# modelscope/FunCodec

Hardware: NVIDIA H100
Metric: codec frames/sec (encode+RVQ+decode) (higher is better)
Workload: dtype f32

## Files before the change

funcodec_b200/csrc/conv_tc.cu:

```cuda
#include <cuda.h>
#include "common.cuh"
#include "kernels.h"
#include "tc_sm90.cuh"
#include <stdlib.h>

namespace fcb {

using namespace tc;

constexpr int TC_M = 128;
constexpr int TC_KC = 32;
constexpr int TC_THREADS = 640;
constexpr int TC_RAW_MAX = 8;
constexpr int TC_PROD = 128;
constexpr int TC_PROWS = TC_PROD / 8;
constexpr int TC_A_ROWS_MAX = 144;
constexpr int TC_GROUP_MMAS = 48;
constexpr int TC_LAUNCH_REGS = 96, TC_PROD_REGS = 96, TC_CTL_REGS = 64, TC_CONS_REGS = 112;
static_assert(128 * (2 * TC_CONS_REGS + 2 * TC_PROD_REGS + TC_CTL_REGS) <= TC_THREADS * TC_LAUNCH_REGS, "register pool");

__device__ __forceinline__ float elu_fast(float v) { return v > 0.f ? v : (__expf(v) - 1.0f); }
__device__ __forceinline__ float elu_scaled(float vs, float k, float s) { return vs > 0.f ? vs : fmaf(exp2f_approx(vs * k), s, -s); }

struct TcSmemLayout {
    int a_rows;
    int a_stage;
    int b_stage;
    int na, nb;
    int nraw, raw_slot, raw_in1, raw_cf;
    int off_b, off_raw, off_bar, total;
};

__host__ __device__ inline TcSmemLayout tc_layout(int K, int S, int n_tile, int na, int nb, int nraw = 0, int raw_pitch = 128,
                                                   int has1 = 0) {
    TcSmemLayout L;
    const int qmax = (K - 1) / S;
    L.a_rows = ((TC_M + qmax + 7) / 8) * 8;
    L.a_stage = 2 * L.a_rows * 128;
    L.b_stage = 2 * n_tile * 128;
    L.na = na; L.nb = nb;
    L.off_b = na * L.a_stage;
    L.nraw = nraw;
    L.raw_in1 = L.a_rows * raw_pitch;
    L.raw_cf = (1 + has1) * L.a_rows * raw_pitch;
    L.raw_slot = (L.raw_cf + 512 + 127) / 128 * 128;
    L.off_raw = L.off_b + nb * L.b_stage;
    L.off_bar = L.off_raw + nraw * L.raw_slot;
    L.total = L.off_bar + 8 * (2 * na + 2 * nb + 2 * TC_RAW_MAX) + 160;
    return L;
}

__host__ __device__ inline int tc_units_per_group(int K, int S, int group_mmas) {
    const int taps = (K + S - 1) / S;
    int g = group_mmas / (12 * taps);
    return g < 1 ? 1 : g;
}

struct TcArgs {
    TcSmemLayout L;
    int na, nb, n_tiles, w_resident, nraw;
    int n_chunks, n_sc, split, n_units, upg, n_groups, n_tt, n_nt, units_per_tile, tq_rows, raw_pitch;
};

struct TcTile { int b, nt, tt; };

__device__ __forceinline__ TcTile tc_tile(int id, int n_nt, int n_tt) {
    TcTile t;
    t.nt = id % n_nt;
    const int r = id / n_nt;
    t.tt = r % n_tt;
    t.b = r / n_tt;
    return t;
}

template <int N_TILE, int KSTEPS>
__device__ __forceinline__ void tc_issue_tap(float (&acc)[N_TILE / 2], uint32_t a_hi, uint32_t a_lo, uint32_t b_hi, uint32_t b_lo,
                                             uint32_t accum) {
    wgmma_fence();
#pragma unroll
    for (int ks = 0; ks < KSTEPS; ++ks) {
        WgmmaF16<N_TILE>::mma(acc, make_desc_k_sw128(a_lo + ks * 32), make_desc_k_sw128(b_hi + ks * 32), ks == 0 ? accum : 1u);
        WgmmaF16<N_TILE>::mma(acc, make_desc_k_sw128(a_hi + ks * 32), make_desc_k_sw128(b_lo + ks * 32), 1u);
        WgmmaF16<N_TILE>::mma(acc, make_desc_k_sw128(a_hi + ks * 32), make_desc_k_sw128(b_hi + ks * 32), 1u);
    }
    wgmma_commit();
}

template <int N_TILE, bool FREQ>
__global__ void __launch_bounds__(TC_THREADS, 1) conv1d_tc_kernel(const __grid_constant__ ConvParams p, const __grid_constant__ TcArgs ka,
                                                                 const __grid_constant__ CUtensorMap tm0,
                                                                 const __grid_constant__ CUtensorMap tm1) {
    extern __shared__ __align__(1024) uint8_t smem_raw[];
    const int tid = threadIdx.x, lane = tid & 31, warp = tid >> 5;
    const int C_in = p.C_in, K = p.K, S = p.S;
    const bool has1 = p.in1.x != nullptr;
    const TcSmemLayout& L = ka.L;
#define na_stages ka.na
#define nb_stages ka.nb
#define n_tiles ka.n_tiles
#define w_resident ka.w_resident
#define nraw ka.nraw
#define raw_pitch ka.raw_pitch
#define n_chunks ka.n_chunks
#define n_sc ka.n_sc
#define n_units ka.n_units
#define upg ka.upg
#define n_groups ka.n_groups
#define n_tt ka.n_tt
#define n_nt ka.n_nt
    const bool split = ka.split != 0;

    uint8_t* smA = smem_raw;
    uint8_t* smB = smem_raw + L.off_b;
    uint64_t* bars = reinterpret_cast<uint64_t*>(smem_raw + L.off_bar);
    uint64_t* a_full = bars;
    uint64_t* a_empty = a_full + na_stages;
    uint64_t* b_full = a_empty + na_stages;
    uint64_t* b_empty = b_full + nb_stages;
    uint64_t* raw_full = b_empty + nb_stages;
    uint64_t* raw_empty = raw_full + TC_RAW_MAX;
    double* red = reinterpret_cast<double*>(raw_empty + TC_RAW_MAX);
    uint8_t* smR = smem_raw + L.off_raw;
#define units_per_tile ka.units_per_tile
#define tq_rows ka.tq_rows
    auto tile_interior = [&](int t0) -> bool {
        if (nraw == 0) return false;
        const int t_last = (t0 + TC_M < p.T_out ? t0 + TC_M : p.T_out) - 1;
        const int lo = t0 * S - p.pad_l;
        const int hi = t_last * S - p.pad_l + (K - 1);
        return lo >= 0 && hi < tq_rows * S;
    };

    if (tid == 0) {
        for (int i = 0; i < na_stages; ++i) { mbar_init(a_full + i, split ? 2 * TC_PROD : TC_PROD); mbar_init(a_empty + i, 2); }
        for (int i = 0; i < nb_stages; ++i) { mbar_init(b_full + i, 1); mbar_init(b_empty + i, 2); }
        for (int i = 0; i < TC_RAW_MAX; ++i) { mbar_init(raw_full + i, 1); mbar_init(raw_empty + i, TC_PROD); }
        mbar_fence_init();
    }
    __syncthreads();

    const int role = warp >> 2;
    if (role < 2) {
        setmaxnreg_dec<TC_PROD_REGS>();
        const int grp = role;
        const int ptid = tid & (TC_PROD - 1);
        const int jchunk = ptid & 7;
        const int wq = (ptid >> 5), lq = (lane >> 3);
        const int rsub = ((wq >> 1) << 3) + ((wq & 1) << 1) + (lq & 1) + ((lq >> 1) << 2);
        constexpr int NR = TC_A_ROWS_MAX / TC_PROWS;
        const int gt_max = (p.T_out - 1) * S - p.pad_l + (K - 1);
        const int step = split ? 1 : 2;
        const int half = split ? grp : 0;
        int tile = blockIdx.x, unit = split ? 0 : grp;
        int as = unit % na_stages;
        uint32_t aphase = 0;
        const float in_scale = p.tc_in_scale;
        int rawbase = 0;
        while (unit >= n_units && tile < n_tiles) {
            if (tile_interior(tc_tile(tile, n_nt, n_tt).tt * TC_M)) rawbase += units_per_tile;
            unit -= n_units; tile += gridDim.x;
        }
        while (tile < n_tiles) {
            const TcTile tl = tc_tile(tile, n_nt, n_tt);
            const int t0 = tl.tt * TC_M;
            int b = tl.b, f_out = 0;
            if (FREQ) { b = tl.b / p.fq.F_out; f_out = tl.b - b * p.fq.F_out; }
            const int pitch = FREQ ? p.fq.cin : C_in;
            const float* x0 = p.in0.x + (long long)b * p.in0.clip_stride + (long long)p.in0.row_off * pitch;
            const float* x1 = has1 ? p.in1.x + (long long)b * p.in1.clip_stride + (long long)p.in1.row_off * pitch : nullptr;
            const float* cf0 = p.in0.coef ? p.in0.coef + (long long)b * 2 * pitch : nullptr;
            const float* cf1 = (has1 && p.in1.coef) ? p.in1.coef + (long long)b * 2 * pitch : nullptr;
            const int cur_tile = tile;
            const bool interior = tile_interior(t0);
            for (; unit < n_units && tile == cur_tile; ) {
                const int sc = unit / S, ph = unit - sc * S;
                const int chunk = 2 * sc + half;
                const uint32_t par = aphase ^ 1;
                uint8_t* hi = smA + as * L.a_stage;
                uint8_t* lo = hi + L.a_rows * 128;
                const uint32_t c16 = (uint32_t)(half * 4 + (jchunk >> 1)), sub8 = (uint32_t)((jchunk & 1) << 3);
                if (p.dbg & 512) {
                    if (p.dbg & 64) mbar_wait(a_empty + as, par); else mbar_wait_backoff(a_empty + as, par, 64);
                } else if (chunk >= n_chunks) {
                    if (p.dbg & 64) mbar_wait(a_empty + as, par); else mbar_wait_backoff(a_empty + as, par, 64);
                } else if (interior) {
// ... 109 lines not shown
#pragma unroll
                    for (int j = 0; j < PB; ++j) {
                        const int u = rsub + TC_PROWS * (i0 + j);
                        if (u < L.a_rows) {
                            float4 v = make_float4(0.f, 0.f, 0.f, 0.f);
                            if (p.dbg & 2) v = xa[j];
                            else if (okr[j]) {
                                const float4 xv = xa[j];
                                v.x = fmaf(xv.x, a0.x, b0.x); v.y = fmaf(xv.y, a0.y, b0.y);
                                v.z = fmaf(xv.z, a0.z, b0.z); v.w = fmaf(xv.w, a0.w, b0.w);
                                if (has1) {
                                    const float4 yv = xb[j];
                                    v.x = v.x + fmaf(yv.x, a1.x, b1.x); v.y = v.y + fmaf(yv.y, a1.y, b1.y);
                                    v.z = v.z + fmaf(yv.z, a1.z, b1.z); v.w = v.w + fmaf(yv.w, a1.w, b1.w);
                                }
                                if (p.elu) {
                                    v.x = elu_scaled(v.x, p.tc_elu_k, in_scale); v.y = elu_scaled(v.y, p.tc_elu_k, in_scale);
                                    v.z = elu_scaled(v.z, p.tc_elu_k, in_scale); v.w = elu_scaled(v.w, p.tc_elu_k, in_scale);
                                }
                            }
                            if (p.dbg & 4) continue;
                            uint2 h, l;
                            split_f16x2(v.x, v.y, h.x, l.x);
                            split_f16x2(v.z, v.w, h.y, l.y);
                            const uint32_t o = (uint32_t)u * 128u + ((c16 ^ (uint32_t)(u & 7)) << 4) + sub8;
                            *reinterpret_cast<uint2*>(hi + o) = h;
                            *reinterpret_cast<uint2*>(lo + o) = l;
                        }
                    }
                }
                fence_proxy_async_smem();
                }
                mbar_arrive(a_full + as);
                as += step;
                if (as >= na_stages) { as -= na_stages; aphase ^= 1; }
                unit += step;
            }
            while (unit >= n_units && tile < n_tiles) {
                if (tile_interior(tc_tile(tile, n_nt, n_tt).tt * TC_M)) rawbase += units_per_tile;
                unit -= n_units; tile += gridDim.x;
            }
        }
    } else if (role == 2) {
        setmaxnreg_dec<TC_CTL_REGS>();
        if (warp == 8 && lane == 0) {
            const uint32_t bytes = (uint32_t)L.b_stage;
            int bs = 0;
            uint32_t bphase = 0;
            bool first = true;
            for (int tile = blockIdx.x; tile < n_tiles; tile += gridDim.x) {
                if (w_resident && !first) break;
                const TcTile tl = tc_tile(tile, n_nt, n_tt);
                const uint8_t* wbase = reinterpret_cast<const uint8_t*>(p.w_tc) + (long long)tl.nt * n_sc * K * bytes;
                int chunk = 0, ph = 0;
                for (int unit = 0; unit < n_units; ++unit) {
                    for (int k = ph; k < K; k += S) {
                        if (!w_resident) { if (p.dbg & 64) mbar_wait(b_empty + bs, bphase ^ 1); else mbar_wait_backoff(b_empty + bs, bphase ^ 1, 64); }
                        if (p.dbg & 256) { mbar_arrive(b_full + bs); }
                        else {
                            mbar_arrive_expect_tx(b_full + bs, bytes);
                            bulk_g2s(smB + bs * L.b_stage, wbase + ((long long)chunk * K + k) * bytes, bytes, b_full + bs);
                        }
                        if (++bs == nb_stages) { bs = 0; bphase ^= 1; }
                    }
                    if (++ph == S) { ph = 0; ++chunk; }
                }
                first = false;
            }
        } else if (warp == 9 && lane == 0 && nraw > 0 && !(p.dbg & 512)) {
            const uint32_t row_bytes = (uint32_t)(L.a_rows * raw_pitch);
            const uint32_t cbytes = (uint32_t)raw_pitch;
            const uint32_t n_cf = (p.in0.coef ? 2u : 0u) + ((has1 && p.in1.coef) ? 2u : 0u);
            const uint32_t unit_bytes = row_bytes * (has1 ? 2u : 1u) + n_cf * cbytes;
            int rc = 0;
            for (int tile = blockIdx.x; tile < n_tiles; tile += gridDim.x) {
                const TcTile tl = tc_tile(tile, n_nt, n_tt);
                const int t0 = tl.tt * TC_M;
                if (!tile_interior(t0)) continue;
                int b = tl.b, f_out = 0;
                if (FREQ) { b = tl.b / p.fq.F_out; f_out = tl.b - b * p.fq.F_out; }
                const int pitch = FREQ ? p.fq.cin : C_in;
                const float* cf0 = p.in0.coef ? p.in0.coef + (long long)b * 2 * pitch : nullptr;
                const float* cf1 = (has1 && p.in1.coef) ? p.in1.coef + (long long)b * 2 * pitch : nullptr;
                for (int sc = 0; sc < n_sc; ++sc)
                    for (int ph = 0; ph < S; ++ph) {
                        const int r = ph - p.pad_l;
                        const int fd = (r >= 0) ? r / S : -((-r + S - 1) / S);
                        const int tq0 = t0 + fd, php = r - fd * S;
                        for (int hh = 0; hh < 2; ++hh) {
                            const int chunk = 2 * sc + hh;
                            if (chunk >= n_chunks) break;
                            const int slot = rc % nraw;
                            mbar_wait(raw_empty + slot, (uint32_t)((rc / nraw) & 1) ^ 1);
                            uint8_t* dst = smR + slot * L.raw_slot;
                            mbar_arrive_expect_tx(raw_full + slot, unit_bytes);
                            int c0 = chunk * TC_KC;
                            if (FREQ) {
                                const int kf = c0 / pitch;
                                c0 -= kf * pitch;
                                int f_src = f_out * p.fq.SF + kf - p.fq.pad_f;
                                if (!p.pad_zero) f_src = reflect_index(f_src, p.fq.F_in);
                                tma_load_5d(dst, &tm0, c0, php, tq0, f_src, b, raw_full + slot);
                                if (has1) tma_load_5d(dst + L.raw_in1, &tm1, c0, php, tq0, f_src, b, raw_full + slot);
                            } else {
                                tma_load_4d(dst, &tm0, c0, php, tq0, b, raw_full + slot);
                                if (has1) tma_load_4d(dst + L.raw_in1, &tm1, c0, php, tq0, b, raw_full + slot);
                            }
                            if (cf0) {
                                bulk_g2s(dst + L.raw_cf, cf0 + c0, cbytes, raw_full + slot);
                                bulk_g2s(dst + L.raw_cf + 128, cf0 + pitch + c0, cbytes, raw_full + slot);
                            }
                            if (cf1) {
                                bulk_g2s(dst + L.raw_cf + 256, cf1 + c0, cbytes, raw_full + slot);
                                bulk_g2s(dst + L.raw_cf + 384, cf1 + pitch + c0, cbytes, raw_full + slot);
                            }
                            ++rc;
                        }
                    }
            }
        }
    } else {
        setmaxnreg_inc<TC_CONS_REGS>();
        constexpr int NA = N_TILE / 2;
        const int cw = warp - 12;
        const int wg = cw >> 2;
        const int ctid = tid - 12 * 32;
        const bool leader = (tid & 127) == 0;
        const uint32_t a_base = smem_u32(smA) + (uint32_t)(wg * 64 * 128), b_base = smem_u32(smB);
        const int r_lo = wg * 64 + (cw & 3) * 16 + (lane >> 2);
        const int cq = 2 * (lane & 3);
        const bool plain_out = FREQ && p.fq.FR == 1 && p.fq.TR == 1 && p.fq.c_store == p.C_out;
        const float out_scale = p.tc_out_scale;
        int fin_clip = -1, fin_local = 0;
        auto fin_flush = [&]() {
            if (fin_clip < 0 || fin_local == 0) return;
            int* flag = reinterpret_cast<int*>(red + 16);
            if (ctid == 0) {
                __threadfence();
                const int old = atomicAdd(p.fin_counter + fin_clip, fin_local);
                *flag = (old + fin_local == p.fin_parts) ? 1 : 0;
            }
            asm volatile("bar.sync 1, 256;" ::: "memory");
            const bool last_cta = *flag != 0;
            if (last_cta) {
                __threadfence();
                const double* pp = p.partials + (long long)fin_clip * p.fin_parts * 2;
                double fs = 0.0, fss = 0.0;
                for (int i = ctid; i < p.fin_parts; i += 256) { fs += __ldcg(pp + 2 * i); fss += __ldcg(pp + 2 * i + 1); }
#pragma unroll
                for (int o = 16; o > 0; o >>= 1) {
                    fs += __shfl_xor_sync(0xffffffffu, fs, o);
                    fss += __shfl_xor_sync(0xffffffffu, fss, o);
                }
                asm volatile("bar.sync 1, 256;" ::: "memory");
                if (lane == 0) { red[cw * 2] = fs; red[cw * 2 + 1] = fss; }
                asm volatile("bar.sync 1, 256;" ::: "memory");
                double ts = 0.0, tss = 0.0;
#pragma unroll
                for (int w = 0; w < 8; ++w) { ts += red[2 * w]; tss += red[2 * w + 1]; }
                const double mean_d = ts / p.fin_count;
                double var = tss / p.fin_count - mean_d * mean_d;
                if (var < 0.0) var = 0.0;
                const float mean = (float)mean_d, rstd = (float)(1.0 / sqrt(var + (double)p.fin_eps));
                if (ctid == 0) {
                    p.fin_stats[2 * fin_clip] = mean;
                    p.fin_stats[2 * fin_clip + 1] = rstd;
                    p.fin_counter[fin_clip] = 0;
                }
                if (p.fin_coef)
// ... 29 lines not shown
                        const uint32_t b_hi0 = b_base + bs * L.b_stage;
                        const uint32_t b_lo0 = b_hi0 + N_TILE * 128;
                        if (full_stage) tc_issue_tap<N_TILE, 4>(acc, a_hi0 + q * 128, a_lo0 + q * 128, b_hi0, b_lo0, accum);
                        else tc_issue_tap<N_TILE, 2>(acc, a_hi0 + q * 128, a_lo0 + q * 128, b_hi0, b_lo0, accum);
                        accum = 1;
                        wgmma_wait<1>();
                        mbar_arrive_if(b_empty + pend_b, leader && pend_b >= 0);
                        mbar_arrive_if(a_empty + pend_a, leader && pend_a >= 0);
                        pend_b = w_resident ? -1 : bs;
                        pend_a = -1;
                        if (++bs == nb_stages) { bs = 0; bphase ^= 1; }
                    }
                    pend_a = as;
                    if (++as == na_stages) { as = 0; aphase ^= 1; }
                    if (++ph == S) ph = 0;
                }
                wgmma_wait<0>();
                reg_fence(acc);
                if (leader) {
                    if (pend_b >= 0) mbar_arrive(b_empty + pend_b);
                    if (pend_a >= 0) mbar_arrive(a_empty + pend_a);
                }
                pend_a = -1; pend_b = -1;
#pragma unroll
                for (int i = 0; i < NA; ++i) tot[i] = g == 0 ? acc[i] : tot[i] + acc[i];
            }
            first = false;
            long long frow = 0;
            if (FREQ) {
                const int fb = tl.b / p.fq.F_out, ff = tl.b - fb * p.fq.F_out;
                frow = ((long long)fb * p.fq.F_out * p.fq.FR + (long long)ff * p.fq.FR) * ((long long)p.T_out * p.fq.TR);
            }
            const float* bias = p.bias + tl.nt * N_TILE;
            float s = 0.f, ss = 0.f;
#pragma unroll
            for (int j = 0; j < N_TILE / 8; ++j) {
                const int c = 8 * j + cq;
                const float bias0 = __ldg(bias + c), bias1 = __ldg(bias + c + 1);
#pragma unroll
                for (int h = 0; h < 2; ++h) {
                    const int t = tl.tt * TC_M + r_lo + 8 * h;
                    if (t >= p.T_out) continue;
                    float2 o;
                    o.x = fmaf(tot[4 * j + 2 * h], out_scale, bias0);
                    o.y = fmaf(tot[4 * j + 2 * h + 1], out_scale, bias1);
                    s += o.x + o.y;
                    ss = fmaf(o.x, o.x, ss); ss = fmaf(o.y, o.y, ss);
                    if (p.dbg & 8) continue;
                    if (!FREQ || plain_out) {
                        *reinterpret_cast<float2*>(p.out + (long long)tl.b * p.out_clip_stride + (long long)t * p.C_out + tl.nt * N_TILE + c) = o;
                    } else {
#pragma unroll
                        for (int e = 0; e < 2; ++e) {
                            const int co = tl.nt * N_TILE + c + e;
                            const int phs = co / p.fq.Cc, cch = co - phs * p.fq.Cc;
                            if (cch < p.fq.c_store) {
                                const int pf = phs / p.fq.TR, pt = phs - pf * p.fq.TR;
                                p.out[(frow + (long long)t * p.fq.TR + (long long)pf * p.T_out * p.fq.TR + pt) * p.fq.c_store + cch] = e ? o.y : o.x;
                            }
                        }
                    }
                }
            }
            if (p.partials && !(p.dbg & 16)) {
                double ds = (double)s, dss = (double)ss;
#pragma unroll
                for (int o = 16; o > 0; o >>= 1) {
                    ds += __shfl_xor_sync(0xffffffffu, ds, o);
                    dss += __shfl_xor_sync(0xffffffffu, dss, o);
                }
                asm volatile("bar.sync 1, 256;" ::: "memory");
                if (lane == 0) { red[cw * 2] = ds; red[cw * 2 + 1] = dss; }
                asm volatile("bar.sync 1, 256;" ::: "memory");
                if (ctid == 0) {
                    const int nparts = n_nt * n_tt;
                    double* dst = p.partials + ((long long)tl.b * nparts + tl.nt * n_tt + tl.tt) * 2;
                    double ts = 0.0, tss = 0.0;
#pragma unroll
                    for (int w = 0; w < 8; ++w) { ts += red[2 * w]; tss += red[2 * w + 1]; }
                    dst[0] = ts;
                    dst[1] = tss;
                }
                if (p.fin_counter) {
                    const int clip = FREQ ? tl.b / p.fq.F_out : tl.b;
                    if (clip != fin_clip) { fin_flush(); fin_clip = clip; }
                    ++fin_local;
                }
            }
        }
        if (p.fin_counter && p.partials && !(p.dbg & 16)) fin_flush();
    }
#undef na_stages
#undef nb_stages
#undef n_tiles
#undef w_resident
#undef nraw
#undef raw_pitch
#undef n_chunks
#undef n_sc
#undef n_units
#undef upg
#undef n_groups
#undef n_tt
#undef n_nt
#undef units_per_tile
#undef tq_rows
}

bool conv_tc_supported(int C_in, int C_out_eff, int K, int S, int D) {
    return D == 1 && (C_in % TC_KC == 0 || C_in == 16) && C_out_eff % 16 == 0 && K >= 1 && S >= 1 && ((K - 1) / S) <= 16;
}

bool conv_tc_supported_2d(int cin, int C_out_eff, int KT, int ST) {
    const bool cin_ok = cin % 4 == 0 && (cin % TC_KC == 0 || TC_KC % cin == 0);
    return cin_ok && C_out_eff % 16 == 0 && KT >= 1 && ST >= 1 && ((KT - 1) / ST) <= 16;
}

int conv_tc_n_tile(int C_out_eff) {
    if (C_out_eff % 64 == 0) return 64;
    if (C_out_eff % 32 == 0) return 32;
    return 16;
}

int conv_tc_num_parts(int T_out, int C_out_eff) {
    return ((T_out + TC_M - 1) / TC_M) * (C_out_eff / conv_tc_n_tile(C_out_eff));
}

static int g_num_sms = 0;

static int g_group_mmas = TC_GROUP_MMAS, g_deep_ring = 1, g_dbg = 0, g_na_tma = 2;

struct TcPlan { int resident, na, nb, nraw; TcSmemLayout L; bool ok; };

static TcPlan tc_plan(const ConvParams& p, int na_first, bool want_raw, int g_deep_ring) {
    const int limit = 225 * 1024;
    const int n_slabs = ((p.C_in + 2 * TC_KC - 1) / (2 * TC_KC)) * p.K;
    const int has1 = p.in1.x ? 1 : 0;
    const int cin_row = p.fq.KF > 0 ? p.fq.cin : p.C_in;
    const int raw_pitch = (cin_row < TC_KC ? cin_row : TC_KC) * 4;
    TcPlan pl{};
    pl.ok = false;
    int na = na_first, nb = 4;
    TcSmemLayout L = tc_layout(p.K, p.S, p.n_tile, na, n_slabs);
    const int min_raw = want_raw ? 2 : 0;
    auto fits = [&](const TcSmemLayout& l) { return l.total + min_raw * tc_layout(p.K, p.S, p.n_tile, 2, 2, 1, raw_pitch, has1).raw_slot <= limit; };
    if (n_slabs <= 64 && p.C_out == p.n_tile && fits(L)) { pl.resident = 1; nb = n_slabs; }
    else {
        L = tc_layout(p.K, p.S, p.n_tile, na, nb);
        if (!fits(L)) { nb = 3; L = tc_layout(p.K, p.S, p.n_tile, na, nb); }
        if (!fits(L)) { na = 2; nb = 4; L = tc_layout(p.K, p.S, p.n_tile, na, nb); }
        if (!fits(L)) { nb = 3; L = tc_layout(p.K, p.S, p.n_tile, na, nb); }
        if (!fits(L)) { nb = 2; L = tc_layout(p.K, p.S, p.n_tile, na, nb); }
        if (!fits(L)) return pl;
        if (g_deep_ring && !want_raw)
            while (nb < 24 && nb < n_slabs && tc_layout(p.K, p.S, p.n_tile, na, nb + 1).total <= limit)
                L = tc_layout(p.K, p.S, p.n_tile, na, ++nb);
    }
    int nraw = 0;
// ... 31 lines not shown
    const cuuint64_t dims[5] = {(cuuint64_t)cin, (cuuint64_t)ST, (cuuint64_t)(T_in / ST), (cuuint64_t)F_in, (cuuint64_t)B};
    const cuuint64_t strides[4] = {(cuuint64_t)cin * 4, (cuuint64_t)ST * cin * 4, (cuuint64_t)T_raw * cin * 4,
                                   (cuuint64_t)v.clip_stride * 4};
    const cuuint32_t box[5] = {(cuuint32_t)(cin < TC_KC ? cin : TC_KC), 1, (cuuint32_t)a_rows, 1, 1};
    const cuuint32_t estr[5] = {1, 1, 1, 1, 1};
    if (((uintptr_t)base & 15) != 0 || (strides[0] & 15) || (strides[2] & 15) || (strides[3] & 15) || dims[2] == 0) return false;
    return g_encode_tiled(tm, CU_TENSOR_MAP_DATA_TYPE_FLOAT32, 5, const_cast<float*>(base), dims, strides, box, estr,
                          CU_TENSOR_MAP_INTERLEAVE_NONE, CU_TENSOR_MAP_SWIZZLE_NONE, CU_TENSOR_MAP_L2_PROMOTION_L2_128B,
                          CU_TENSOR_MAP_FLOAT_OOB_FILL_NONE) == CUDA_SUCCESS;
}

template <int N_TILE, bool FREQ>
static cudaError_t launch_tc_n(const ConvParams& p, cudaStream_t st, const TcPlan& pl, int n_tiles, const CUtensorMap& tm0,
                               const CUtensorMap& tm1) {
    auto kern = conv1d_tc_kernel<N_TILE, FREQ>;
    {
        cudaError_t e = ensure_dynamic_smem((const void*)kern, 225 * 1024);
        if (e != cudaSuccess) return e;
    }
    const int grid = n_tiles < g_num_sms ? n_tiles : g_num_sms;
    TcArgs ka{};
    ka.L = pl.L; ka.na = pl.na; ka.nb = pl.nb; ka.n_tiles = n_tiles; ka.w_resident = pl.resident; ka.nraw = pl.nraw;
    ka.n_chunks = (p.C_in + TC_KC - 1) / TC_KC;
    ka.n_sc = (ka.n_chunks + 1) >> 1;
    ka.split = ka.n_chunks > 1;
    ka.n_units = ka.n_sc * p.S;
    ka.upg = tc_units_per_group(p.K, p.S, g_group_mmas);
    ka.n_groups = (ka.n_units + ka.upg - 1) / ka.upg;
    ka.n_tt = (p.T_out + TC_M - 1) / TC_M;
    ka.n_nt = p.C_out / N_TILE;
    ka.units_per_tile = ka.n_chunks * p.S;
    ka.tq_rows = p.T_in / p.S;
    ka.raw_pitch = ((FREQ ? p.fq.cin : p.C_in) < TC_KC ? (FREQ ? p.fq.cin : p.C_in) : TC_KC) * 4;
    kern<<<grid, TC_THREADS, pl.L.total, st>>>(p, ka, tm0, tm1);
    return cudaGetLastError();
}

template <int N_TILE>
static cudaError_t launch_tc_modes(const ConvParams& p, cudaStream_t st, const TcPlan& pl, int n_tiles, bool freq,
                                   const CUtensorMap& tm0, const CUtensorMap& tm1) {
    return freq ? launch_tc_n<N_TILE, true>(p, st, pl, n_tiles, tm0, tm1) : launch_tc_n<N_TILE, false>(p, st, pl, n_tiles, tm0, tm1);
}

cudaError_t launch_conv_tc(const ConvParams& p_in, int B, cudaStream_t st, int* nparts) {
    ConvParams p = p_in;
    if (g_num_sms == 0) {
        int dev = 0;
        cudaError_t e = cudaGetDevice(&dev);
        if (e != cudaSuccess) return e;
        e = cudaDeviceGetAttribute(&g_num_sms, cudaDevAttrMultiProcessorCount, dev);
        if (e != cudaSuccess) return e;
        if (const char* v = getenv("FCB_TC_GROUP_MMAS")) g_group_mmas = atoi(v) > 0 ? atoi(v) : TC_GROUP_MMAS;
        if (const char* v = getenv("FCB_TC_DEEP_RING")) g_deep_ring = atoi(v) != 0;
        if (const char* v = getenv("FCB_TC_DBG")) g_dbg = atoi(v);
        if (const char* v = getenv("FCB_TC_NA_TMA")) { const int f = atoi(v); if (f == 2 || f == 4) g_na_tma = f; }
        g_tma_state = -1;
        const char* tv = getenv("FCB_TC_TMA");
        if (!tv || atoi(tv) != 0) {
            void* fn = nullptr;
            cudaDriverEntryPointQueryResult qres;
            if (cudaGetDriverEntryPoint("cuTensorMapEncodeTiled", &fn, cudaEnableDefault, &qres) == cudaSuccess && fn &&
                qres == cudaDriverEntryPointSuccess) {
                g_encode_tiled = (EncodeTiledFn)fn;
                g_tma_state = 1;
            }
        }
    }
    p.dbg = g_dbg;
    if (!(p.tc_in_scale > 0.f)) p.tc_in_scale = 16.f;
    if (!(p.tc_w_scale > 0.f)) p.tc_w_scale = 1.f;
    p.tc_out_scale = 1.0f / (p.tc_in_scale * p.tc_w_scale);
    p.tc_elu_k = 1.4426950408889634f / p.tc_in_scale;
    const int n_tt = (p.T_out + TC_M - 1) / TC_M, n_nt = p.C_out / p.n_tile;
    *nparts = n_tt * n_nt;
    const int n_tiles = n_tt * n_nt * B;
    const bool freq = p.fq.KF > 0;
    CUtensorMap tm0{}, tm1{};
    bool want_raw = g_tma_state == 1 && (n_tt >= 3 || (p.K == 1 && p.S == 1 && p.pad_l == 0)) && p.T_in / p.S >= 1 &&
                    (freq ? (p.fq.cin % TC_KC == 0 || (p.fq.cin == 16 && p.fq.KF == 1)) : (p.C_in % TC_KC == 0 || p.C_in == 16));
    if (freq && !(getenv("FCB_TC_TMA2D") && atoi(getenv("FCB_TC_TMA2D")) != 0)) want_raw = false;
    TcPlan pl{};
    if (want_raw) {
        pl = tc_plan(p, g_na_tma, true, g_deep_ring);
        want_raw = pl.ok && pl.nraw >= 2;
        if (want_raw && !freq)
            want_raw = make_act_map(&tm0, p.in0, p.C_in, p.S, p.T_in, B, pl.L.a_rows) &&
                       (!p.in1.x || make_act_map(&tm1, p.in1, p.C_in, p.S, p.T_in, B, pl.L.a_rows));
        if (want_raw && freq) {
            const int nclips = B / p.fq.F_out;
            want_raw = make_act_map_2d(&tm0, p.in0, p.fq.cin, p.S, p.T_in, p.fq.F_in, p.fq.T_raw0, p.fq.f_off0, nclips, pl.L.a_rows) &&
                       (!p.in1.x || make_act_map_2d(&tm1, p.in1, p.fq.cin, p.S, p.T_in, p.fq.F_in, p.fq.T_raw1, p.fq.f_off1, nclips, pl.L.a_rows));
        }
    }
    if (!want_raw) {
        pl = tc_plan(p, 4, false, g_deep_ring);
        if (!pl.ok) return cudaErrorInvalidConfiguration;
    }
    switch (p.n_tile) {
        case 16: return launch_tc_modes<16>(p, st, pl, n_tiles, freq, tm0, tm1);
        case 32: return launch_tc_modes<32>(p, st, pl, n_tiles, freq, tm0, tm1);
        case 64: return launch_tc_modes<64>(p, st, pl, n_tiles, freq, tm0, tm1);
        default: return cudaErrorInvalidConfiguration;
    }
}

}
```

funcodec_b200/csrc/engine.cu:

```cuda
#include <cuda_runtime.h>
#include <math.h>
#include <stdio.h>
#include <stdlib.h>
#include <string.h>

#include <map>
#include <string>
#include <vector>

#include "../../include/funcodec_b200.h"
#include "common.cuh"
#include "kernels.h"

using namespace fcb;

namespace {

struct HostTensor {
    std::vector<int64_t> shape;
    std::vector<float> data;
};

struct ConvW {
    int cin = 0, cout = 0, k = 0, s = 1, d = 1;
// ... 201 lines not shown
                    }
            }
}

void build_tc_image_tf32(const std::vector<float>& wp , int K, int cin, int cout_eff, int n_tile,
                          std::vector<float>* img_out) {
    const int n_chunks = (cin + 31) / 32, n_nt = cout_eff / n_tile;
    const size_t slab = (size_t)n_tile * 32;
    std::vector<float>& img = *img_out;
    img.assign((size_t)n_nt * n_chunks * K * 2 * slab, 0.f);
    for (int nt = 0; nt < n_nt; ++nt)
        for (int c = 0; c < n_chunks; ++c)
            for (int k = 0; k < K; ++k) {
                float* hi = img.data() + (((size_t)nt * n_chunks + c) * K + k) * 2 * slab;
                float* lo = hi + slab;
                for (int n = 0; n < n_tile; ++n)
                    for (int col = 0; col < 32; ++col) {
                        const float x = (c * 32 + col < cin) ? wp[((size_t)k * cin + c * 32 + col) * cout_eff + nt * n_tile + n] : 0.f;
                        uint32_t u;
                        memcpy(&u, &x, 4);
                        u = (u + 0x1000u) & 0xFFFFE000u;
                        float xh;
                        memcpy(&xh, &u, 4);
                        const size_t off = (size_t)n * 32 + ((((col >> 2) ^ (n & 7)) << 2) | (col & 3));
                        hi[off] = xh;
                        lo[off] = x - xh;
                    }
            }
}

int pack_tc(fcb_handle* h, const std::vector<float>& wp , int K, int cin, int cout_eff, ConvW* o) {
    o->n_tile = 0;
    if (!h->use_tc || !conv_tc_supported(cin, cout_eff, K, 1, o->d)) return FCB_OK;
    const int n_tile = conv_tc_n_tile(cout_eff);
    std::vector<float> img;
    build_tc_image_f16(wp, K, cin, cout_eff, n_tile, &img, &o->tc_scale);
    FCB_TRY(upload(h, img, &o->w_tc));
    o->n_tile = n_tile;
    return FCB_OK;
}

int effective_weight(fcb_handle* h, const std::string& base, std::vector<int64_t> shape, std::vector<float>* w_out) {
    const HostTensor* w = find(h, base + ".weight");
    if (h->cfg.norm == 0 || w) {
        FCB_TRY(need(h, base + ".weight", shape, &w));
        *w_out = w->data;
        return FCB_OK;
    }
    const HostTensor *g, *v;
    FCB_TRY(need(h, base + ".weight_g", {shape[0], 1, 1}, &g));
    FCB_TRY(need(h, base + ".weight_v", shape, &v));
    const size_t inner = (size_t)(shape[1] * shape[2]);
    w_out->resize(v->data.size());
    for (int64_t i = 0; i < shape[0]; ++i) {
        double ss = 0.0;
        for (size_t j = 0; j < inner; ++j) { const double x = v->data[(size_t)i * inner + j]; ss += x * x; }
        const float f = g->data[(size_t)i] / (float)sqrt(ss);
        for (size_t j = 0; j < inner; ++j) (*w_out)[(size_t)i * inner + j] = v->data[(size_t)i * inner + j] * f;
    }
    return FCB_OK;
}

int pack_norm_affine(fcb_handle* h, const std::string& base, int cout, ConvW* o) {
    o->gamma = o->beta = nullptr;
    if (h->cfg.norm != 0) return FCB_OK;
    const HostTensor *g, *be;
    FCB_TRY(need(h, base + ".weight", {cout}, &g));
// ... 369 lines not shown
        const int nres = (int)(h->dec_rb.size() / h->dec_up.size());
        FCB_TRY(run_resblock(r, u, h->dec_rb[i * nres], &sc, &blk));
        FCB_TRY(release(r, u));
        for (int j = 1; j < nres; ++j) {
            Act sc2, blk2;
            FCB_TRY(run_resblock(r, sc, h->dec_rb[i * nres + j], &sc2, &blk2, &blk));
            FCB_TRY(release(r, sc));
            FCB_TRY(release(r, blk));
            sc = sc2; blk = blk2;
        }
        have_blk = true;
    }
    Act f;
    FCB_TRY(run_conv(r, sc, have_blk ? &blk : nullptr, true, nullptr, h->dec_final, true, &f));
    FCB_TRY(release(r, sc));
    if (have_blk) FCB_TRY(release(r, blk));
    FCB_CK(launch_final_output(f.p, f.stats, f.gamma, f.beta, scale, r.B, f.T, out_len, wav_out, r.st));
    h->launches++;
    FCB_TRY(release(r, f));
    FCB_TRY(phase_end(r));
    return FCB_OK;
}

typedef fcb_handle::Conv2W Conv2W;
typedef fcb_handle::ResBlock2W ResBlock2W;

int pack_tc2d(fcb_handle* h, const std::vector<float>& wp, const std::vector<float>& bias, int cout_eff, Conv2W* o) {
    o->n_tile = 0; o->tc_class = 0;
    const int ck = o->kf_eff * o->cin, kt = o->kt_eff;
    const int cout_tc = (cout_eff + 15) / 16 * 16;
    if (!h->use_tc || !conv_tc_supported_2d(o->cin, cout_tc, kt, o->transposed ? 1 : o->st)) return FCB_OK;
    if (cout_tc != cout_eff && o->transposed) return FCB_OK;
    std::vector<float> img;
    const int n_tile = conv_tc_n_tile(cout_tc);
    if (cout_tc == cout_eff) {
        build_tc_image_f16(wp, kt, ck, cout_eff, n_tile, &img, &o->tc_scale);
        o->bias_tc = nullptr;
    } else {
        std::vector<float> wpad((size_t)kt * ck * cout_tc, 0.f), bpad(cout_tc, 0.f);
        for (size_t r = 0; r < (size_t)kt * ck; ++r)
            for (int co = 0; co < cout_eff; ++co) wpad[r * cout_tc + co] = wp[r * cout_eff + co];
        for (int co = 0; co < cout_eff; ++co) bpad[co] = bias[co];
        build_tc_image_f16(wpad, kt, ck, cout_tc, n_tile, &img, &o->tc_scale);
        FCB_TRY(upload(h, bpad, &o->bias_tc));
    }
    FCB_TRY(upload(h, img, &o->w_tc));
    o->n_tile = n_tile; o->cout_tc = cout_tc;
    o->tc_class = cout_tc != cout_eff ? 4 : (o->cin % 32 == 0 ? 1 : 2);
    return FCB_OK;
}

int pack_conv2d(fcb_handle* h, const std::string& prefix, int cin, int cout, int kf, int kt, int sf, int st, Conv2W* o,
                int cin_store = 0, int groups = 1) {
    if (cin_store < cin) cin_store = cin;
    if (groups < 1 || cin % groups != 0 || cout % groups != 0)
        return fail(h, FCB_E_INVALID, "conv groups do not divide the channels of " + prefix + " (check conv_group_ratio)");
    const int cig = cin / groups, cog = cout / groups;
    const HostTensor *w, *b, *g, *be;
    FCB_TRY(need(h, prefix + ".conv.conv.weight", {cout, cig, kf, kt}, &w));
    FCB_TRY(need(h, prefix + ".conv.conv.bias", {cout}, &b));
    FCB_TRY(need(h, prefix + ".conv.norm.weight", {cout}, &g));
    FCB_TRY(need(h, prefix + ".conv.norm.bias", {cout}, &be));
    std::vector<float> p((size_t)kt * kf * cin_store * cout, 0.f);
    for (int co = 0; co < cout; ++co) {
        const int ci0 = (co / cog) * cig;
        for (int cl = 0; cl < cig; ++cl)
            for (int a = 0; a < kf; ++a)
// ... 315 lines not shown
        h->launches += 3;
        FCB_TRY(pool_free(r, Y));
    } else {
        FCB_CK(launch_istft(f.p, f.coef, r.B, f.F_raw, f.T_raw, c.n_fft, c.stft_hop, f.T, scale, frames, wav_out, out_len, r.st));
        h->launches += 2;
    }
    FCB_TRY(pool_free(r, frames));
    FCB_TRY(release2(r, f));
    FCB_TRY(phase_end(r));
    return FCB_OK;
}

int pack_stft_bases(fcb_handle* h) {
    const fcb_config& c = h->cfg;
    const int N = c.n_fft, hop = c.stft_hop, n_bins = N / 2 + 1;
    h->stft_w.n_tile = 0; h->istft_w.n_tile = 0;
    if (!h->use_tc || N % 32 != 0 || hop % 32 != 0 || N < hop) return FCB_OK;
    const double two_pi = 6.283185307179586476925286766559;
    std::vector<double> hann(N);
    for (int n = 0; n < N; ++n) hann[n] = 0.5 - 0.5 * cos(two_pi * n / N);
    {
        const int K = N / 32, cout = (2 * n_bins + 127) / 128 * 128;
        if (!conv_tc_supported(32, cout, K, hop / 32, 1)) return FCB_OK;
        std::vector<float> wp((size_t)K * 32 * cout, 0.f), bias(cout, 0.f);
        for (int n = 0; n < N; ++n)
            for (int k = 0; k < n_bins; ++k) {
                const double ang = two_pi * (double)(((long long)k * n) % N) / N;
                wp[(size_t)n * cout + k] = (float)(hann[n] * cos(ang));
                wp[(size_t)n * cout + n_bins + k] = (float)(-hann[n] * sin(ang));
            }
        ConvW& o = h->stft_w;
        o.cin = 32; o.cout = cout; o.k = K; o.s = hop / 32;
        std::vector<float> img;
        const int n_tile = conv_tc_n_tile(cout);
        build_tc_image_f16(wp, K, 32, cout, n_tile, &img, &o.tc_scale);
        FCB_TRY(upload(h, img, &o.w_tc));
        FCB_TRY(upload(h, bias, &o.bias));
        o.n_tile = n_tile;
        h->stft_ld = cout;
    }
    {
        const int cin = (2 * n_bins + 31) / 32 * 32, cout = N;
        if (!conv_tc_supported(cin, cout, 1, 1, 1)) return FCB_OK;
        std::vector<float> wp((size_t)cin * cout, 0.f), bias(cout, 0.f);
        for (int k = 0; k < n_bins; ++k) {
            const bool edge = (k == 0 || k == N / 2);
            for (int j = 0; j < N; ++j) {
                const double ang = two_pi * (double)(((long long)k * j) % N) / N;
                wp[(size_t)k * cout + j] = (float)((edge ? 1.0 : 2.0) * cos(ang) * hann[j] / N);
                wp[(size_t)(n_bins + k) * cout + j] = edge ? 0.f : (float)(-2.0 * sin(ang) * hann[j] / N);
            }
        }
        ConvW& o = h->istft_w;
        o.cin = cin; o.cout = cout; o.k = 1; o.s = 1;
        std::vector<float> img;
        const int n_tile = conv_tc_n_tile(cout);
        build_tc_image_f16(wp, 1, cin, cout, n_tile, &img, &o.tc_scale);
        FCB_TRY(upload(h, img, &o.w_tc));
        FCB_TRY(upload(h, bias, &o.bias));
        o.n_tile = n_tile;
        h->istft_ld = cin;
    }
    return FCB_OK;
}

int run_plain_tc(Run& r, const float* x, int T_in, const ConvW& L, int T_out, float* out) {
    fcb_handle* h = r.h;
    ConvParams p{};
    p.in0.x = x; p.in0.clip_stride = (long long)T_in * L.cin;
    p.T_in = T_in; p.C_in = L.cin; p.K = L.k; p.S = L.s; p.D = 1; p.pad_l = 0; p.T_ext = T_in; p.pad_zero = 1;
    p.w_tc = L.w_tc; p.n_tile = L.n_tile; p.tc_w_scale = L.tc_scale; p.bias = L.bias;
    p.out = out; p.T_out = T_out; p.C_out = L.cout; p.out_clip_stride = (long long)T_out * L.cout;
    int np = 0;
    FCB_CK(launch_conv_tc(p, r.B, r.st, &np));
    h->launches++;
    return FCB_OK;
}

int finalize_freq(fcb_handle* h) {
    const fcb_config& c = h->cfg;
    const int nf = c.n_filters, D = c.dimension, nr = c.n_ratios;
    FCB_TRY(pack_conv2d(h, "encoder.model.0", 3, nf, c.kernel_size, c.kernel_size, 1, 1, &h->f_enc_conv0, 4));
    int n = 1, mult = 1;
    for (int i = nr - 1; i >= 0; --i) {
        const int fr = c.ratios_f[i], tr = c.ratios[i];
        ResBlock2W rb; Conv2W down;
        FCB_TRY(pack_resblock2d(h, "encoder.model." + std::to_string(n), mult * nf, &rb));
        FCB_TRY(pack_conv2d(h, "encoder.model." + std::to_string(n + 2), mult * nf, 2 * mult * nf, 2 * fr, 2 * tr, fr, tr, &down, 0,
                            conv_groups_of(mult * nf, c.conv_group_ratio)));
// ... 677 lines not shown
```

funcodec_b200/csrc/kernels.h:

```cpp
#pragma once
#include <cuda_runtime.h>
#include <stdint.h>
#include "common.cuh"

namespace fcb {

cudaError_t ensure_dynamic_smem(const void* kernel, int bytes);

void conv_pick_tile(int T_out, int C_out, int C_in, int K, int B, int* tx, int* tm, bool* two);
int conv_num_parts(int T_out, int C_out, int C_in, int K, int B);
cudaError_t launch_conv(const ConvParams& p, int B, cudaStream_t st, int* nparts);
cudaError_t launch_stats_finalize(const double* partials, int nparts, double count, float eps, int mode,
                                  float* out, int B, cudaStream_t st, const float* gamma = nullptr,
                                  const float* beta = nullptr, int C = 0, float* coef = nullptr);
bool conv_cout1_supported(const ConvParams& p);
int conv_cout1_num_parts(int T_out);
cudaError_t launch_conv_cout1(const ConvParams& p, int B, cudaStream_t st, int* nparts);
int sumsq_num_parts(int L);
cudaError_t launch_sumsq_partials(const float* x, int B, int L, double* partials, int* nparts, cudaStream_t st);

bool conv_tc_supported(int C_in, int C_out_eff, int K, int S, int D);
bool conv_tc_supported_2d(int cin, int C_out_eff, int KT, int ST);
int conv_tc_n_tile(int C_out_eff);
int conv_tc_num_parts(int T_out, int C_out_eff);
cudaError_t launch_conv_tc(const ConvParams& p, int B, cudaStream_t st, int* nparts);

int conv2d_num_parts(const Conv2dParams& p);
cudaError_t launch_conv2d(const Conv2dParams& p, cudaStream_t st);
bool conv2d_small_cout_supported(const Conv2dParams& p);
int conv2d_small_cout_num_parts(const Conv2dParams& p);
cudaError_t launch_conv2d_small_cout(const Conv2dParams& p, cudaStream_t st);
cudaError_t launch_stft_magphase(const float* wav, const float* scale, int B, int L, int n_fft, int hop, int n_frames,
                                 int cpad, float* feats, cudaStream_t st);
cudaError_t launch_istft(const float* raw, const float* coef, int B, int F_raw, int T_raw, int n_fft, int hop, int n_frames,
                         const float* scale, float* frames, float* out, int out_len, cudaStream_t st);

cudaError_t launch_wave_rows(const float* wav, const float* scale, int B, int L, int n_fft, int n_rows, float* rows, cudaStream_t st);
cudaError_t launch_magphase_from_spec(const float* spec, int ld, int B, int n_bins, int n_frames, int cpad, float* feats,
                                      cudaStream_t st);
cudaError_t launch_spec_rows(const float* raw, const float* coef, int B, int F_raw, int T_raw, int n_bins, int n_frames, int ld,
                             float* Y, cudaStream_t st);
cudaError_t launch_istft_ola(const float* frames, const float* scale, int B, int n_fft, int hop, int n_frames, int out_len,
                             float* out, cudaStream_t st);

struct LstmSeqParams {
    const float* gx;
    const float* whh;
    float* h_seq;
    float* y_out;
    InView skip;
    unsigned* barrier;
    int B, T, H;
    int fast_cell;
    float whh_scale, whh_inv_scale;
    unsigned long long* trace;
};
// ... 42 lines not shown
```

Measured before the change: 121,700.

## Add 128-wide N tile to tensor-core conv with one producer warpgroup

Adds an N_TILE=128 variant of the warp-specialized wgmma conv kernel for non-frequency convs whose output channel count is a multiple of 128. Role counts, thread count and register budgets are templated per tile width: a single producer warpgroup handles both halves of split A loads, and consumers get more registers for the larger accumulator. The norm partial statistics are still emitted per 64-column part, so downstream partial counts do not change. The aim is more reuse of each A tile per wgmma and fewer tiles per layer. The cost is higher register pressure and possibly less producer throughput with only one producer group.

```diff
diff --git a/funcodec_b200/csrc/conv_tc.cu b/funcodec_b200/csrc/conv_tc.cu
--- a/funcodec_b200/csrc/conv_tc.cu
+++ b/funcodec_b200/csrc/conv_tc.cu
@@ -10,14 +10,22 @@
 
 constexpr int TC_M = 128;
 constexpr int TC_KC = 32;
-constexpr int TC_THREADS = 640;
 constexpr int TC_RAW_MAX = 8;
 constexpr int TC_PROD = 128;
 constexpr int TC_PROWS = TC_PROD / 8;
 constexpr int TC_A_ROWS_MAX = 144;
 constexpr int TC_GROUP_MMAS = 48;
-constexpr int TC_LAUNCH_REGS = 96, TC_PROD_REGS = 96, TC_CTL_REGS = 64, TC_CONS_REGS = 112;
-static_assert(128 * (2 * TC_CONS_REGS + 2 * TC_PROD_REGS + TC_CTL_REGS) <= TC_THREADS * TC_LAUNCH_REGS, "register pool");
+template <int N_TILE>
+struct TcRoles {
+    static constexpr int PROD_GROUPS = N_TILE > 64 ? 1 : 2;
+    static constexpr int THREADS = 128 * (PROD_GROUPS + 3);
+    static constexpr int LAUNCH_REGS = 65536 / THREADS / 8 * 8;
+    static constexpr int PROD_REGS = N_TILE > 64 ? 112 : 96, CTL_REGS = 64, CONS_REGS = N_TILE > 64 ? 168 : 112;
+    static constexpr int CTL_WG = PROD_GROUPS;
+    static constexpr int CONS_WG = PROD_GROUPS + 1;
+    static constexpr int PARTS = N_TILE > 64 ? N_TILE / 64 : 1;
+    static_assert(128 * (2 * CONS_REGS + PROD_GROUPS * PROD_REGS + CTL_REGS) <= THREADS * LAUNCH_REGS, "register pool");
+};
 
 __device__ __forceinline__ float elu_fast(float v) { return v > 0.f ? v : (__expf(v) - 1.0f); }
 __device__ __forceinline__ float elu_scaled(float vs, float k, float s) { return vs > 0.f ? vs : fmaf(exp2f_approx(vs * k), s, -s); }
@@ -46,7 +54,7 @@
     L.raw_slot = (L.raw_cf + 512 + 127) / 128 * 128;
     L.off_raw = L.off_b + nb * L.b_stage;
     L.off_bar = L.off_raw + nraw * L.raw_slot;
-    L.total = L.off_bar + 8 * (2 * na + 2 * nb + 2 * TC_RAW_MAX) + 160;
+    L.total = L.off_bar + 8 * (2 * na + 2 * nb + 2 * TC_RAW_MAX) + 128 * (n_tile > 64 ? n_tile / 64 : 1) + 32;
     return L;
 }
 
@@ -87,9 +95,10 @@
 }
 
 template <int N_TILE, bool FREQ>
-__global__ void __launch_bounds__(TC_THREADS, 1) conv1d_tc_kernel(const __grid_constant__ ConvParams p, const __grid_constant__ TcArgs ka,
+__global__ void __launch_bounds__(TcRoles<N_TILE>::THREADS, 1) conv1d_tc_kernel(const __grid_constant__ ConvParams p, const __grid_constant__ TcArgs ka,
                                                                  const __grid_constant__ CUtensorMap tm0,
                                                                  const __grid_constant__ CUtensorMap tm1) {
+    using R = TcRoles<N_TILE>;
     extern __shared__ __align__(1024) uint8_t smem_raw[];
     const int tid = threadIdx.x, lane = tid & 31, warp = tid >> 5;
     const int C_in = p.C_in, K = p.K, S = p.S;
@@ -140,8 +149,8 @@
     __syncthreads();
 
     const int role = warp >> 2;
-    if (role < 2) {
-        setmaxnreg_dec<TC_PROD_REGS>();
+    if (role < R::PROD_GROUPS) {
+        setmaxnreg_dec<R::PROD_REGS>();
         const int grp = role;
         const int ptid = tid & (TC_PROD - 1);
         const int jchunk = ptid & 7;
@@ -149,8 +158,9 @@
         const int rsub = ((wq >> 1) << 3) + ((wq & 1) << 1) + (lq & 1) + ((lq >> 1) << 2);
         constexpr int NR = TC_A_ROWS_MAX / TC_PROWS;
         const int gt_max = (p.T_out - 1) * S - p.pad_l + (K - 1);
-        const int step = split ? 1 : 2;
-        const int half = split ? grp : 0;
+        const int step = split ? 1 : R::PROD_GROUPS;
+        const int half0 = (split && R::PROD_GROUPS == 2) ? grp : 0;
+        int half = half0;
         int tile = blockIdx.x, unit = split ? 0 : grp;
         int as = unit % na_stages;
         uint32_t aphase = 0;
@@ -326,6 +336,8 @@
                 fence_proxy_async_smem();
                 }
                 mbar_arrive(a_full + as);
+                if (R::PROD_GROUPS == 1 && split && half == 0) { half = 1; continue; }
+                half = half0;
                 as += step;
                 if (as >= na_stages) { as -= na_stages; aphase ^= 1; }
                 unit += step;
@@ -335,9 +347,9 @@
                 unit -= n_units; tile += gridDim.x;
             }
         }
-    } else if (role == 2) {
-        setmaxnreg_dec<TC_CTL_REGS>();
-        if (warp == 8 && lane == 0) {
+    } else if (role == R::CTL_WG) {
+        setmaxnreg_dec<R::CTL_REGS>();
+        if (warp == 4 * R::CTL_WG && lane == 0) {
             const uint32_t bytes = (uint32_t)L.b_stage;
             int bs = 0;
             uint32_t bphase = 0;
@@ -361,7 +373,7 @@
                 }
                 first = false;
             }
-        } else if (warp == 9 && lane == 0 && nraw > 0 && !(p.dbg & 512)) {
+        } else if (warp == 4 * R::CTL_WG + 1 && lane == 0 && nraw > 0 && !(p.dbg & 512)) {
             const uint32_t row_bytes = (uint32_t)(L.a_rows * raw_pitch);
             const uint32_t cbytes = (uint32_t)raw_pitch;
             const uint32_t n_cf = (p.in0.coef ? 2u : 0u) + ((has1 && p.in1.coef) ? 2u : 0u);
@@ -414,11 +426,12 @@
             }
         }
     } else {
-        setmaxnreg_inc<TC_CONS_REGS>();
+        setmaxnreg_inc<R::CONS_REGS>();
         constexpr int NA = N_TILE / 2;
-        const int cw = warp - 12;
+        constexpr int PARTS = R::PARTS;
+        const int cw = warp - 4 * R::CONS_WG;
         const int wg = cw >> 2;
-        const int ctid = tid - 12 * 32;
+        const int ctid = tid - 128 * R::CONS_WG;
         const bool leader = (tid & 127) == 0;
         const uint32_t a_base = smem_u32(smA) + (uint32_t)(wg * 64 * 128), b_base = smem_u32(smB);
         const int r_lo = wg * 64 + (cw & 3) * 16 + (lane >> 2);
@@ -428,7 +441,7 @@
         int fin_clip = -1, fin_local = 0;
         auto fin_flush = [&]() {
             if (fin_clip < 0 || fin_local == 0) return;
-            int* flag = reinterpret_cast<int*>(red + 16);
+            int* flag = reinterpret_cast<int*>(red + 16 * PARTS);
             if (ctid == 0) {
                 __threadfence();
                 const int old = atomicAdd(p.fin_counter + fin_clip, fin_local);
@@ -524,10 +537,13 @@
                 frow = ((long long)fb * p.fq.F_out * p.fq.FR + (long long)ff * p.fq.FR) * ((long long)p.T_out * p.fq.TR);
             }
             const float* bias = p.bias + tl.nt * N_TILE;
-            float s = 0.f, ss = 0.f;
+            float s[PARTS], ss[PARTS];
+#pragma unroll
+            for (int hp = 0; hp < PARTS; ++hp) { s[hp] = 0.f; ss[hp] = 0.f; }
 #pragma unroll
             for (int j = 0; j < N_TILE / 8; ++j) {
                 const int c = 8 * j + cq;
+                const int hp = j * PARTS / (N_TILE / 8);
                 const float bias0 = __ldg(bias + c), bias1 = __ldg(bias + c + 1);
 #pragma unroll
                 for (int h = 0; h < 2; ++h) {
@@ -536,8 +552,8 @@
                     float2 o;
                     o.x = fmaf(tot[4 * j + 2 * h], out_scale, bias0);
                     o.y = fmaf(tot[4 * j + 2 * h + 1], out_scale, bias1);
-                    s += o.x + o.y;
-                    ss = fmaf(o.x, o.x, ss); ss = fmaf(o.y, o.y, ss);
+                    s[hp] += o.x + o.y;
+                    ss[hp] = fmaf(o.x, o.x, ss[hp]); ss[hp] = fmaf(o.y, o.y, ss[hp]);
                     if (p.dbg & 8) continue;
                     if (!FREQ || plain_out) {
                         *reinterpret_cast<float2*>(p.out + (long long)tl.b * p.out_clip_stride + (long long)t * p.C_out + tl.nt * N_TILE + c) = o;
@@ -555,28 +571,36 @@
                 }
             }
             if (p.partials && !(p.dbg & 16)) {
-                double ds = (double)s, dss = (double)ss;
-#pragma unroll
-                for (int o = 16; o > 0; o >>= 1) {
-                    ds += __shfl_xor_sync(0xffffffffu, ds, o);
-                    dss += __shfl_xor_sync(0xffffffffu, dss, o);
+                double ds[PARTS], dss[PARTS];
+#pragma unroll
+                for (int hp = 0; hp < PARTS; ++hp) {
+                    ds[hp] = (double)s[hp]; dss[hp] = (double)ss[hp];
+#pragma unroll
+                    for (int o = 16; o > 0; o >>= 1) {
+                        ds[hp] += __shfl_xor_sync(0xffffffffu, ds[hp], o);
+                        dss[hp] += __shfl_xor_sync(0xffffffffu, dss[hp], o);
+                    }
                 }
                 asm volatile("bar.sync 1, 256;" ::: "memory");
-                if (lane == 0) { red[cw * 2] = ds; red[cw * 2 + 1] = dss; }
+                if (lane == 0) {
+#pragma unroll
+                    for (int hp = 0; hp < PARTS; ++hp) { red[(hp * 8 + cw) * 2] = ds[hp]; red[(hp * 8 + cw) * 2 + 1] = dss[hp]; }
+                }
                 asm volatile("bar.sync 1, 256;" ::: "memory");
-                if (ctid == 0) {
-                    const int nparts = n_nt * n_tt;
-                    double* dst = p.partials + ((long long)tl.b * nparts + tl.nt * n_tt + tl.tt) * 2;
+                if (ctid < PARTS) {
+                    const int hp = ctid;
+                    const int nparts = n_nt * PARTS * n_tt;
+                    double* dst = p.partials + ((long long)tl.b * nparts + (tl.nt * PARTS + hp) * n_tt + tl.tt) * 2;
                     double ts = 0.0, tss = 0.0;
 #pragma unroll
-                    for (int w = 0; w < 8; ++w) { ts += red[2 * w]; tss += red[2 * w + 1]; }
+                    for (int w = 0; w < 8; ++w) { ts += red[(hp * 8 + w) * 2]; tss += red[(hp * 8 + w) * 2 + 1]; }
                     dst[0] = ts;
                     dst[1] = tss;
                 }
                 if (p.fin_counter) {
                     const int clip = FREQ ? tl.b / p.fq.F_out : tl.b;
                     if (clip != fin_clip) { fin_flush(); fin_clip = clip; }
-                    ++fin_local;
+                    fin_local += PARTS;
                 }
             }
         }
@@ -608,14 +632,19 @@
     return cin_ok && C_out_eff % 16 == 0 && KT >= 1 && ST >= 1 && ((KT - 1) / ST) <= 16;
 }
 
-int conv_tc_n_tile(int C_out_eff) {
+static int tc_part_cols(int C_out_eff) {
     if (C_out_eff % 64 == 0) return 64;
     if (C_out_eff % 32 == 0) return 32;
     return 16;
 }
 
+int conv_tc_n_tile(int C_out_eff, bool freq) {
+    if (!freq && C_out_eff % 128 == 0) return 128;
+    return tc_part_cols(C_out_eff);
+}
+
 int conv_tc_num_parts(int T_out, int C_out_eff) {
-    return ((T_out + TC_M - 1) / TC_M) * (C_out_eff / conv_tc_n_tile(C_out_eff));
+    return ((T_out + TC_M - 1) / TC_M) * (C_out_eff / tc_part_cols(C_out_eff));
 }
 
 static int g_num_sms = 0;
@@ -713,7 +742,7 @@
     ka.units_per_tile = ka.n_chunks * p.S;
     ka.tq_rows = p.T_in / p.S;
     ka.raw_pitch = ((FREQ ? p.fq.cin : p.C_in) < TC_KC ? (FREQ ? p.fq.cin : p.C_in) : TC_KC) * 4;
-    kern<<<grid, TC_THREADS, pl.L.total, st>>>(p, ka, tm0, tm1);
+    kern<<<grid, TcRoles<N_TILE>::THREADS, pl.L.total, st>>>(p, ka, tm0, tm1);
     return cudaGetLastError();
 }
 
@@ -753,7 +782,7 @@
     p.tc_out_scale = 1.0f / (p.tc_in_scale * p.tc_w_scale);
     p.tc_elu_k = 1.4426950408889634f / p.tc_in_scale;
     const int n_tt = (p.T_out + TC_M - 1) / TC_M, n_nt = p.C_out / p.n_tile;
-    *nparts = n_tt * n_nt;
+    *nparts = n_tt * (p.C_out / tc_part_cols(p.C_out));
     const int n_tiles = n_tt * n_nt * B;
     const bool freq = p.fq.KF > 0;
     CUtensorMap tm0{}, tm1{};
@@ -781,6 +810,7 @@
         case 16: return launch_tc_modes<16>(p, st, pl, n_tiles, freq, tm0, tm1);
         case 32: return launch_tc_modes<32>(p, st, pl, n_tiles, freq, tm0, tm1);
         case 64: return launch_tc_modes<64>(p, st, pl, n_tiles, freq, tm0, tm1);
+        case 128: return freq ? cudaErrorInvalidConfiguration : launch_tc_n<128, false>(p, st, pl, n_tiles, tm0, tm1);
         default: return cudaErrorInvalidConfiguration;
     }
 }
diff --git a/funcodec_b200/csrc/engine.cu b/funcodec_b200/csrc/engine.cu
--- a/funcodec_b200/csrc/engine.cu
+++ b/funcodec_b200/csrc/engine.cu
@@ -257,7 +257,7 @@
 int pack_tc(fcb_handle* h, const std::vector<float>& wp , int K, int cin, int cout_eff, ConvW* o) {
     o->n_tile = 0;
     if (!h->use_tc || !conv_tc_supported(cin, cout_eff, K, 1, o->d)) return FCB_OK;
-    const int n_tile = conv_tc_n_tile(cout_eff);
+    const int n_tile = conv_tc_n_tile(cout_eff, false);
     std::vector<float> img;
     build_tc_image_f16(wp, K, cin, cout_eff, n_tile, &img, &o->tc_scale);
     FCB_TRY(upload(h, img, &o->w_tc));
@@ -693,7 +693,7 @@
     if (!h->use_tc || !conv_tc_supported_2d(o->cin, cout_tc, kt, o->transposed ? 1 : o->st)) return FCB_OK;
     if (cout_tc != cout_eff && o->transposed) return FCB_OK;
     std::vector<float> img;
-    const int n_tile = conv_tc_n_tile(cout_tc);
+    const int n_tile = conv_tc_n_tile(cout_tc, true);
     if (cout_tc == cout_eff) {
         build_tc_image_f16(wp, kt, ck, cout_eff, n_tile, &img, &o->tc_scale);
         o->bias_tc = nullptr;
@@ -1075,7 +1075,7 @@
         ConvW& o = h->stft_w;
         o.cin = 32; o.cout = cout; o.k = K; o.s = hop / 32;
         std::vector<float> img;
-        const int n_tile = conv_tc_n_tile(cout);
+        const int n_tile = conv_tc_n_tile(cout, false);
         build_tc_image_f16(wp, K, 32, cout, n_tile, &img, &o.tc_scale);
         FCB_TRY(upload(h, img, &o.w_tc));
         FCB_TRY(upload(h, bias, &o.bias));
@@ -1097,7 +1097,7 @@
         ConvW& o = h->istft_w;
         o.cin = cin; o.cout = cout; o.k = 1; o.s = 1;
         std::vector<float> img;
-        const int n_tile = conv_tc_n_tile(cout);
+        const int n_tile = conv_tc_n_tile(cout, false);
         build_tc_image_f16(wp, 1, cin, cout, n_tile, &img, &o.tc_scale);
         FCB_TRY(upload(h, img, &o.w_tc));
         FCB_TRY(upload(h, bias, &o.bias));
diff --git a/funcodec_b200/csrc/kernels.h b/funcodec_b200/csrc/kernels.h
--- a/funcodec_b200/csrc/kernels.h
+++ b/funcodec_b200/csrc/kernels.h
@@ -21,7 +21,7 @@
 
 bool conv_tc_supported(int C_in, int C_out_eff, int K, int S, int D);
 bool conv_tc_supported_2d(int cin, int C_out_eff, int KT, int ST);
-int conv_tc_n_tile(int C_out_eff);
+int conv_tc_n_tile(int C_out_eff, bool freq);
 int conv_tc_num_parts(int T_out, int C_out_eff);
 cudaError_t launch_conv_tc(const ConvParams& p, int B, cudaStream_t st, int* nparts);
 
```

After: 132,600, median of 6. 1.09x the previous value.
